# zhaoyuhsin/Edge-Guided-Near-Eye-Image-Analysis-for-Head-Mounted-Displays

Hardware: AMD Instinct MI355X
Metric: eye-frames/sec (320x240): inference edge+seg (value), +fit, exact fp32, and train fwd+bwd at 1 MI355X (higher is better)
Workload: dtype f32 tensors; inference products split into f16 hi/lo pairs (3 f16 MFMAs per product, 22-bit significand), f32 accumulate (`exact_fp32`: every product on the f32 MFMA); `train`: bf16 storage, f32 accumulate, f32 master weights (and an f32-storage leg)

## Files before the change

edge-guided-near-eye-image-analysis-for-head-mounted-displays_amd/_lib.py:

```python
import ctypes as C
import os

_HERE = os.path.dirname(os.path.abspath(__file__))
LIB_PATH = os.environ.get("EGNE_LIB") or os.path.join(_HERE, "csrc", "libegne_hip.so")

MAXSEG, MAXGROUP = 8, 3
ACT_NONE, ACT_RELU, ACT_LEAKY = 0, 1, 2

c_fp = C.c_void_p


class Seg(C.Structure):
    _fields_ = [("ptr", c_fp), ("pix_stride", C.c_int64), ("ch_off", C.c_int32), ("Cp", C.c_int32),
                ("scale", c_fp), ("shift", c_fp), ("act_in", C.c_int32), ("presplit", C.c_int32)]


class ConvDesc(C.Structure):
    _fields_ = [("B", C.c_int32), ("H", C.c_int32), ("W", C.c_int32), ("Ho", C.c_int32), ("Wo", C.c_int32),
                ("kh", C.c_int32), ("kw", C.c_int32), ("stride", C.c_int32),
                ("pad_h", C.c_int32), ("pad_w", C.c_int32), ("pad_mode", C.c_int32),
                ("ngroups", C.c_int32), ("dil", C.c_int32 * MAXGROUP),
                ("nseg", C.c_int32), ("seg", Seg * MAXSEG),
                ("Ktot", C.c_int32), ("CoutP", C.c_int32),
                ("w", c_fp), ("bias", c_fp), ("act", C.c_int32),
                ("post_scale", c_fp), ("post_shift", c_fp),
                ("residual", c_fp), ("res_pix_stride", C.c_int64), ("res_ch_off", C.c_int32),
                ("out", c_fp), ("out_pix_stride", C.c_int64), ("out_ch_off", C.c_int32),
                ("Cout_store", C.c_int32),
                ("stats_ws", c_fp), ("stats_nchunk", C.c_int32),
                ("pool_out", c_fp), ("pool_pix_stride", C.c_int64), ("pool_ch_off", C.c_int32),
                ("dyn_scale", C.c_void_p), ("absmax_out", C.c_void_p), ("dtype", C.c_int32),
                ("out_split", C.c_int32), ("out_split_scale", C.c_float), ("ovf_flag", C.c_void_p), ("f16_products", C.c_int32),
                ("mask_y", C.c_void_p), ("mask_pix_stride", C.c_int64), ("mask_ch_off", C.c_int32), ("mask_act", C.c_int32), ("mask_sums", C.c_void_p)]


class Dst(C.Structure):
    _fields_ = [("out", C.c_void_p), ("out_pix_stride", C.c_int64), ("out_ch_off", C.c_int32), ("C", C.c_int32), ("CoutP", C.c_int32),
                ("wfrag", C.c_void_p), ("residual", C.c_void_p), ("res_pix_stride", C.c_int64), ("res_ch_off", C.c_int32),
                ("mask_y", C.c_void_p), ("mask_pix_stride", C.c_int64), ("mask_ch_off", C.c_int32), ("act", C.c_int32),
                ("sums", C.c_void_p), ("res_pixels", C.c_int64)]


MAXDST = 6


class ConvQuery(C.Structure):
    _fields_ = [("dtype", C.c_int32), ("B", C.c_int32), ("H", C.c_int32), ("W", C.c_int32),
                ("kh", C.c_int32), ("kw", C.c_int32), ("stride", C.c_int32), ("pad_h", C.c_int32), ("pad_w", C.c_int32), ("pad_mode", C.c_int32),
                ("ngroups", C.c_int32), ("dil", C.c_int32 * MAXGROUP), ("nseg", C.c_int32),
                ("seg_C", C.c_int32 * MAXSEG), ("seg_Cp", C.c_int32 * MAXSEG), ("seg_ch_off", C.c_int32 * MAXSEG), ("seg_pix_stride", C.c_int64 * MAXSEG),
                ("seg_affine", C.c_int32 * MAXSEG), ("seg_planar", C.c_int32), ("seg_presplit", C.c_int32),
                ("Cout", C.c_int32), ("Cout_store", C.c_int32), ("dst_Cp", C.c_int32), ("dst_ch_off", C.c_int32), ("dst_pix_stride", C.c_int64),
                ("act", C.c_int32), ("has_post", C.c_int32), ("has_residual", C.c_int32), ("res_pix_stride", C.c_int64), ("res_ch_off", C.c_int32),
                ("split", C.c_int32), ("split1", C.c_int32), ("split_c4", C.c_int32), ("train", C.c_int32), ("dyn_scales", C.c_int32),
                ("is_dgrad", C.c_int32), ("want_stats", C.c_int32), ("want_pool", C.c_int32), ("pool_Cp", C.c_int32), ("pool_pix_stride", C.c_int64),
                ("want_scores", C.c_int32), ("up_add", C.c_int32), ("narrow_bf16_ok", C.c_int32), ("f16_products", C.c_int32), ("f16_storage", C.c_int32)]


class ConvChoice(C.Structure):
    _fields_ = [("kind", C.c_int32), ("name", C.c_char * 32), ("tail_frames", C.c_int32), ("fused_stats", C.c_int32), ("fused_pool", C.c_int32),
                ("small_ws_floats", C.c_int64)]


class BdcnTailDesc(C.Structure):
    _fields_ = [("B", C.c_int32), ("H", C.c_int32), ("W", C.c_int32),
                ("s", c_fp * 5), ("s1", c_fp * 5), ("h", C.c_int32 * 5), ("w", C.c_int32 * 5),
                ("stride", C.c_int32 * 5), ("crop", C.c_int32 * 5), ("up", c_fp * 5),
                ("fuse_w", c_fp), ("fuse_b", c_fp), ("out", c_fp * 11), ("edge_thres", C.c_int32)]


class LossDesc(C.Structure):
    _fields_ = [("B", C.c_int32), ("H", C.c_int32), ("W", C.c_int32),
                ("logits", c_fp), ("pix_stride", C.c_int64), ("ch_off", C.c_int32),
                ("target", c_fp), ("spatWts", c_fp), ("distMap", c_fp), ("cond", c_fp),
                ("pupil_center", c_fp), ("elNorm", c_fp), ("elOut", c_fp), ("alpha", C.c_float),
                ("grid_x", c_fp), ("grid_y", c_fp),
                ("partials", c_fp), ("out_terms", c_fp), ("pred_c", c_fp), ("elPred", c_fp),
                ("mask", c_fp), ("op_nchw", c_fp), ("coef", c_fp), ("dtype", C.c_int32),
                ("g_op_nchw", c_fp), ("g_pred_c", c_fp), ("g_elOut_up", c_fp)]


i32, i64, f32, vp = C.c_int32, C.c_int64, C.c_float, C.c_void_p
SIGNATURES = {
    "egne_conv2d_fwd": (i32, [C.POINTER(ConvDesc), vp]),
    "egne_pack_conv_weight": (i32, [vp, i32, i32, i32, i32, vp, i32, i32, vp, vp]),
    "egne_pack_conv_weight_frag": (i32, [vp, i32, i32, i32, i32, vp, i32, i32, vp, vp]),
    "egne_conv3x3_halo_supported": (i32, [C.POINTER(ConvDesc)]),
    "egne_conv3x3_halo_fwd": (i32, [C.POINTER(ConvDesc), vp]),
    "egne_conv3x3_smallcin_fwd": (i32, [C.POINTER(ConvDesc), vp, vp]),
    "egne_pack_conv_weight_f16x2": (i32, [vp, i32, i32, i32, i32, i32, i32, f32, vp, vp, vp]),
    "egne_conv2d_f16x3_fwd": (i32, [C.POINTER(ConvDesc), vp, vp, f32, f32, vp]),
    "egne_conv2d_f16x3_small_workspace_floats": (i64, [C.POINTER(ConvDesc)]),
    "egne_conv2d_f16x3_small_fwd": (i32, [C.POINTER(ConvDesc), vp, vp, f32, f32, vp, i64, vp]),
    "egne_pack_conv_weight_f16frag": (i32, [vp, i32, i32, i32, i32, i32, i32, f32, vp, vp, vp]),
    "egne_conv3x3_halo_f16_fwd": (i32, [C.POINTER(ConvDesc), vp, vp, f32, f32, vp]),
    "egne_conv1x1_3x3_fused_f16_fwd": (i32, [C.POINTER(ConvDesc), C.POINTER(ConvDesc), vp, vp, f32, f32, vp, vp, f32, f32, vp]),
    "egne_conv3x3c4_3x3_fused_f16_fwd": (i32, [C.POINTER(ConvDesc), C.POINTER(ConvDesc), vp, vp, f32, f32, vp, vp, f32, f32, vp]),
    "egne_msblock_dil_scores_f16_fwd": (i32, [C.POINTER(ConvDesc), vp, vp, f32, f32, vp, vp, vp, vp, i32, vp]),
    "egne_msblock_dil_f16_fwd": (i32, [C.POINTER(ConvDesc), vp, vp, f32, f32, vp]),
    "egne_conv3x3_rs_f16_fwd": (i32, [C.POINTER(ConvDesc), vp, vp, f32, f32, vp]),
    "egne_conv3x3_rw_f16_fwd": (i32, [C.POINTER(ConvDesc), vp, vp, f32, f32, vp]),
    "egne_conv1x1_pool2_f16x3_fwd": (i32, [C.POINTER(ConvDesc), vp, vp, f32, f32, vp]),
    "egne_conv1x1_f16x3_fwd": (i32, [C.POINTER(ConvDesc), vp, vp, f32, f32, vp]),
    "egne_dist_maps_workspace_bytes": (i64, [i32, i32, i32, i32]),
    "egne_dist_maps": (i32, [vp, i32, i32, i32, i32, vp, vp, vp]),
    "egne_zscore": (i32, [vp, vp, i32, i32, vp]),
    "egne_spatial_weights": (i32, [vp, i32, i32, i32, vp, vp]),
    "egne_eval_prep_workspace_bytes": (i64, [i32, i32, i32, i32, i32]),
    "egne_eval_prep": (i32, [vp, i32, i32, i32, i32, i32, i32, i32, vp, vp, vp, vp, i32, i32, vp, vp, vp, vp]),
    "egne_eval_render": (i32, [vp, i32, i32, i32, i32, i32, vp, vp, vp, i32, i32, C.c_double, i32, vp, vp, vp, vp, vp]),
    "egne_deepvog_loss_workspace_floats": (i64, [i32, i32, i32]),
    "egne_deepvog_loss_fwd": (i32, [vp, i64, i32, vp, vp, vp, i32, i32, i32, vp, vp, vp, vp, vp, vp]),
    "egne_deepvog_loss_bwd": (i32, [vp, i64, i32, vp, vp, vp, i32, i32, i32, vp, vp, vp, vp, i64, i32, vp]),
    "egne_affine_act": (i32, [vp, i64, i32, vp, i64, i32, i32, i64, vp, vp, i32, vp]),
    "egne_augment": (i32, [vp, vp, vp, vp, vp, vp, vp, vp, i32, i32, i32, vp]),
    "egne_conv3x3_smallcin_f16_fwd": (i32, [C.POINTER(ConvDesc), vp, vp, f32, f32, vp]),
    "egne_pack_conv3x3_c4_weight_f16": (i32, [vp, i32, i32, i32, f32, vp, vp, vp]),
    "egne_conv1x1_ms_f16x3_fwd": (i32, [C.POINTER(ConvDesc), vp, vp, f32, f32, vp]),
    "egne_pack_conv1x1_weight_f16x2_map": (i32, [vp, i32, i32, vp, i32, i32, f32, vp, vp, vp]),
    "egne_conv2d_f16x3_big_fwd": (i32, [C.POINTER(ConvDesc), vp, f32, f32, vp]),
    "egne_pack_conv_weight_f16img": (i32, [vp, i32, i32, i32, i32, i32, i32, f32, vp, vp]),
    "egne_conv2d_f16_big1_fwd": (i32, [C.POINTER(ConvDesc), vp, f32, f32, vp]),
    "egne_conv2d_f16_big1_supported": (i32, [C.POINTER(ConvDesc)]),
    "egne_pack_conv_weight_f16img1": (i32, [vp, i32, i32, i32, i32, i32, i32, f32, vp, vp]),
    "egne_pack_conv1x1_weight_f16": (i32, [vp, i32, i32, vp, i32, i32, f32, vp, vp, vp]),
    "egne_absmax": (i32, [vp, i64, i32, i32, i64, vp, vp]),
    "egne_absmax_f16": (i32, [vp, i64, i32, i32, i64, vp, vp]),
    "egne_norm_stats_workspace_bytes": (i64, [i32, i32, i32, i32]),
    "egne_norm_stats": (i32, [vp, i64, i32, i32, i32, i32, i32, f32, vp, vp, vp, vp, vp, vp]),
    "egne_norm_stats_finish": (i32, [vp, i32, i32, i32, i32, f32, vp, vp, vp]),
    "egne_norm_stats_finish_moments": (i32, [vp, i32, i32, i32, i32, f32, vp, vp, vp, vp, vp]),
    "egne_affine_inplace": (i32, [vp, i64, i32, i32, i64, vp, vp, vp]),
    "egne_affine": (i32, [vp, i64, i32, vp, i64, i32, i32, i64, vp, vp, vp]),
    "egne_avgpool2": (i32, [vp, i64, i32, vp, i64, i32, i32, i32, i32, i32, vp]),
    "egne_norm_act_pool2": (i32, [vp, i64, i32, vp, vp, i32, vp, i64, i32, i32, i32, i32, i32, vp]),
    "egne_maxpool2": (i32, [vp, i64, i32, vp, i64, i32, i32, i32, i32, i32, i32, i32, i32, vp]),
    "egne_maxpool2_f16": (i32, [vp, i64, i32, vp, i64, i32, i32, i32, i32, i32, i32, i32, i32, vp]),
    "egne_maxpool2_split": (i32, [vp, i64, i32, vp, i64, i32, i32, i32, i32, i32, i32, i32, i32, vp]),
    "egne_upsample2x": (i32, [vp, i64, i32, vp, i64, i32, i32, i32, i32, i32, vp]),
    "egne_upsample2x_nearest": (i32, [vp, i64, i32, vp, i64, i32, i32, i32, i32, i32, vp]),
    "egne_upsample2x_nearest_bwd": (i32, [vp, i64, i32, vp, i64, i32, i32, i32, i32, i32, vp]),
    "egne_nchw_to_nhwc": (i32, [vp, i32, i32, i32, i32, vp, i64, i32, i32, vp]),
    "egne_nhwc_to_nchw": (i32, [vp, i64, i32, i32, i32, i32, i32, vp, vp]),
    "egne_bdcn_stage_scores": (i32, [C.POINTER(vp), i32, i64, i64, vp, vp, vp, vp, vp, vp, vp, vp, vp]),
    "egne_bdcn_tail": (i32, [C.POINTER(BdcnTailDesc), vp]),
    "egne_loss_workspace_floats": (i64, [i32, i32, i32]),
    "egne_loss_fwd": (i32, [C.POINTER(LossDesc), vp]),
    "egne_ellipse_head_act": (i32, [vp, i32, i32, vp]),
    "egne_selu_inplace": (i32, [vp, i64, vp]),
    "egne_spatial_mean": (i32, [vp, i64, i32, i32, i32, i32, vp, vp]),
    "egne_softmax3": (i32, [vp, i64, i32, vp, i64, i32, i32, i64, vp]),
    "egne_adain": (i32, [vp, i64, i32, i32, vp, vp, i64, i32, vp, i64, i32, i32, i32, f32, vp]),
    "egne_conf_loss": (i32, [vp, i32, vp, i32, i32, i32, f32, vp, vp]),
    "egne_loss_bwd": (i32, [C.POINTER(LossDesc), vp, vp, i64, i32, vp, vp]),
    "egne_act_bwd_bias_workspace_bytes": (i64, [i64, i32]),
    "egne_act_bwd_bias": (i32, [vp, i64, i32, vp, i64, i32, i32, i32, i64, vp, i32, i32, vp, vp]),
    "egne_act_bwd_bias_absmax": (i32, [vp, i64, i32, vp, i64, i32, i32, i32, i64, vp, i32, i32, vp, vp, vp]),
    "egne_act_norm_bwd": (i32, [vp, i64, i32, vp, i64, i32, i32, vp, vp, vp, i64, i32, vp, i64, i32, i32, i32, i32, i32, i32, vp, vp, vp, i32, vp, i32, vp]),
    "egne_bn_act_bwd": (i32, [vp, i64, i32, i32, vp, vp, vp, vp, i64, i32, i32, i32, i32, i32, vp, i64, i32, vp, vp, vp, vp, i32, vp, i32, vp, vp]),
    "egne_zero_many": (i32, [vp, i32, i64, vp]),
    "egne_pair_bias_bwd_workspace_bytes": (i64, [i32, i32]),
    "egne_pair_bias_bwd": (i32, [vp, i64, i32, i32, i32, i32, i32, vp, vp, i32, i32, vp, vp, vp, vp]),
    "egne_norm_bwd_workspace_bytes": (i64, [i32, i32, i32, i32]),
    "egne_norm_pool2_bwd": (i32, [vp, i64, i32, vp, vp, vp, i64, i32, i32, i32, i32, i32, i32, vp, i64, i32, i32, vp, vp, vp]),
    "egne_norm_bwd_store": (i32, [vp, i64, i32, vp, vp, vp, vp, i64, i32, i32, i32, i32, i32, i32, vp, i64, i32, vp, vp, vp,
                                  i32, vp, vp]),
    "egne_norm_bwd": (i32, [vp, i64, i32, vp, vp, vp, vp, i64, i32, i32, i32, i32, i32, i32, vp, i64, i32, vp, vp, vp,
                            i32, vp, vp]),
    "egne_avgpool2_bwd": (i32, [vp, i64, i32, vp, i64, i32, i32, i32, i32, i32, vp]),
    "egne_upsample2x_bwd": (i32, [vp, i64, i32, vp, i64, i32, i32, i32, i32, i32, vp]),
    "egne_upsample2x_bwd_store": (i32, [vp, i64, i32, vp, i64, i32, i32, i32, i32, i32, vp]),
    "egne_ellipse_head_act_bwd": (i32, [vp, vp, i32, i32, vp]),
    "egne_selu_bwd": (i32, [vp, vp, i64, vp]),
    "egne_softmax3_bwd": (i32, [vp, i64, i32, vp, i64, i32, vp, i64, i32, i64, vp]),
    "egne_adain_bwd": (i32, [vp, i64, i32, i32, vp, i64, i32, vp, i64, i32, vp, i64, i32, vp, vp, i64, i32, i32, i32, f32, vp]),
    "egne_reflect_pad_bwd": (i32, [vp, i64, i32, i32, i32, vp, i64, i32, i32, i32, i32, i32, vp]),
    "egne_spatial_mean_bwd": (i32, [vp, i32, vp, i64, i32, i32, i32, i32, vp]),
    "egne_conf_loss_bwd": (i32, [vp, i32, vp, i32, i32, i32, vp, vp, i32, vp]),
    "egne_conv2d_wgrad_splits": (i32, [C.POINTER(ConvDesc)]),
    "egne_conv2d_wgrad_workspace_bytes": (i64, [C.POINTER(ConvDesc)]),
    "egne_conv2d_wgrad": (i32, [C.POINTER(ConvDesc), vp, i64, i32, i32, i32, vp, C.POINTER(vp), vp, vp]),
# ... 66 lines not shown
```

edge-guided-near-eye-image-analysis-for-head-mounted-displays_amd/csrc/common.h:

```cpp
#pragma once
#include <hip/hip_runtime.h>
#include <cstdarg>
#include <cstdio>
#include <mutex>
#include <unordered_map>
#include "../../include/egne_hip.h"

static __device__ __attribute__((aligned(256), used)) float egne_zero_page[64] = {0};

typedef __bf16 egne_bf16;
typedef float egne_f32x4 __attribute__((ext_vector_type(4)));
typedef __bf16 egne_bf16x4 __attribute__((ext_vector_type(4)));
typedef __bf16 egne_bf16x8 __attribute__((ext_vector_type(8)));

__device__ __forceinline__ egne_f32x4 ld4(const float* p) { return *(const egne_f32x4*)p; }
__device__ __forceinline__ egne_f32x4 ld4(const egne_bf16* p) { return __builtin_convertvector(*(const egne_bf16x4*)p, egne_f32x4); }
__device__ __forceinline__ void st4(float* p, egne_f32x4 v) { *(egne_f32x4*)p = v; }
__device__ __forceinline__ void st4(egne_bf16* p, egne_f32x4 v) { *(egne_bf16x4*)p = __builtin_convertvector(v, egne_bf16x4); }
__device__ __forceinline__ float ld1(const float* p) { return *p; }
__device__ __forceinline__ float ld1(const egne_bf16* p) { return (float)*p; }
__device__ __forceinline__ void st1(float* p, float v) { *p = v; }
__device__ __forceinline__ void st1(egne_bf16* p, float v) { *p = (egne_bf16)v; }
template <typename T> struct egne_vt { static constexpr int N = 4; };
template <> struct egne_vt<egne_bf16> { static constexpr int N = 8; };
template <int N> struct egne_fv { float v[N]; };
__device__ __forceinline__ egne_fv<4> ldv(const float* p) {
  const egne_f32x4 t = *(const egne_f32x4*)p;
  return egne_fv<4>{{t[0], t[1], t[2], t[3]}};
}
__device__ __forceinline__ egne_fv<8> ldv(const egne_bf16* p) {
  typedef unsigned u4_ __attribute__((ext_vector_type(4)));
  const u4_ w = *(const u4_*)p;
  egne_fv<8> r;
#pragma unroll
  for (int i = 0; i < 4; ++i) {
    r.v[2 * i] = __builtin_bit_cast(float, w[i] << 16);
    r.v[2 * i + 1] = __builtin_bit_cast(float, w[i] & 0xffff0000u);
  }
  return r;
}
__device__ __forceinline__ void stv(float* p, const egne_fv<4>& a) { *(egne_f32x4*)p = egne_f32x4{a.v[0], a.v[1], a.v[2], a.v[3]}; }
__device__ __forceinline__ void stv(egne_bf16* p, const egne_fv<8>& a) {
  const egne_f32x4 lo = {a.v[0], a.v[1], a.v[2], a.v[3]}, hi = {a.v[4], a.v[5], a.v[6], a.v[7]};
  const egne_bf16x4 l = __builtin_convertvector(lo, egne_bf16x4), h = __builtin_convertvector(hi, egne_bf16x4);
  *(egne_bf16x8*)p = egne_bf16x8{l[0], l[1], l[2], l[3], h[0], h[1], h[2], h[3]};
}
typedef unsigned egne_u32x4 __attribute__((ext_vector_type(4)));
template <typename T> __device__ __forceinline__ egne_u32x4 ldraw(const T* p) { return *(const egne_u32x4*)p; }
__device__ __forceinline__ egne_fv<4> unpackv(const float*, egne_u32x4 w) {
  return egne_fv<4>{{__builtin_bit_cast(float, w[0]), __builtin_bit_cast(float, w[1]), __builtin_bit_cast(float, w[2]), __builtin_bit_cast(float, w[3])}};
}
__device__ __forceinline__ egne_fv<8> unpackv(const egne_bf16*, egne_u32x4 w) {
  egne_fv<8> r;
#pragma unroll
  for (int i = 0; i < 4; ++i) {
    r.v[2 * i] = __builtin_bit_cast(float, w[i] << 16);
    r.v[2 * i + 1] = __builtin_bit_cast(float, w[i] & 0xffff0000u);
  }
  return r;
}
template <int N> __device__ __forceinline__ egne_fv<N> ldf(const float* p) {
  egne_fv<N> r;
#pragma unroll
  for (int i = 0; i < N; i += 4) { const egne_f32x4 t = *(const egne_f32x4*)(p + i); r.v[i] = t[0]; r.v[i + 1] = t[1]; r.v[i + 2] = t[2]; r.v[i + 3] = t[3]; }
  return r;
}
template <int N> __device__ __forceinline__ egne_fv<N> fv_fill(float x) {
  egne_fv<N> r;
#pragma unroll
  for (int i = 0; i < N; ++i) r.v[i] = x;
  return r;
}
template <typename T> __device__ __forceinline__ const T* zero_page() { return (const T*)egne_zero_page; }

#ifdef EGNE_NO_OVF_CHECK
__device__ __forceinline__ bool egne_nonfinite(float) { return false; }
__device__ __forceinline__ bool egne_nonfinite64(double) { return false; }
#else
__device__ __forceinline__ bool egne_nonfinite(float v) { return __builtin_amdgcn_classf(v, 0x207); }
__device__ __forceinline__ bool egne_nonfinite64(double v) { return !__builtin_isfinite(v); }
#endif
__device__ __forceinline__ bool egne_ovf_row(int y, int H) { return y % 3 == 1 || y == H - 1; }
__device__ __forceinline__ void egne_ovf_commit(bool bad, unsigned* flag) {
  if (flag && bad) atomicOr(flag, 1u);
}

namespace egne {

char* err_buf();

inline int fail(int code, const char* fmt, ...) {
  va_list ap;
  va_start(ap, fmt);
  vsnprintf(err_buf(), 512, fmt, ap);
  va_end(ap);
  return code;
}

inline bool fp32_storage(const egne_conv_desc& d) {
  for (int i = 0; i < d.nseg && i < EGNE_MAXSEG; ++i)
    if (d.seg[i].presplit != 0) return false;
  return d.out_split == 0;
}

inline int check_launch(const char* what) {
  hipError_t e = hipGetLastError();
  if (e != hipSuccess) return fail(EGNE_ERR_LAUNCH, "%s: %s", what, hipGetErrorString(e));
  return EGNE_OK;
}

inline bool raise_lds(const void* kern, size_t bytes) {
  static std::mutex mu;
  static std::unordered_map<const void*, size_t> have;
  std::lock_guard<std::mutex> g(mu);
  auto it = have.find(kern);
  if (it != have.end() && it->second >= bytes) return true;
  if (hipFuncSetAttribute(kern, hipFuncAttributeMaxDynamicSharedMemorySize, (int)bytes) != hipSuccess) {
    (void)hipGetLastError();
    return false;
  }
  have[kern] = bytes;
  return true;
}

#define EGNE_REQUIRE(cond, ...) \
  do { if (!(cond)) return ::egne::fail(EGNE_ERR_ARG, __VA_ARGS__); } while (0)

bool halo3_supported(const egne_conv_desc& d);
int halo3_launch(const egne_conv_desc& d, hipStream_t st);

bool wgrad_halo_supported(const egne_conv_desc& d, long long gzs);
int wgrad_halo_splits(const egne_conv_desc& d);
int wgrad_halo_launch(const egne_conv_desc& d, const float* gz, long long gzs, int gzo, float* ws, hipStream_t st);
int wgrad_halo_f16_launch(const egne_conv_desc& d, const float* gz, long long gzs, int gzo, const unsigned* gz_dyn, float* ws, hipStream_t st);

bool wgrad3x3_bf16_supported(const egne_conv_desc& d, long long gzs);
int wgrad3x3_bf16_splits(const egne_conv_desc& d);
int wgrad3x3_bf16_launch(const egne_conv_desc& d, const egne_bf16* gz, long long gzs, int gzo, float* ws, hipStream_t st);
bool wgrad1x1_bf16_supported(const egne_conv_desc& d, long long gzs);
int wgrad1x1_bf16_splits(const egne_conv_desc& d);
int wgrad1x1_bf16_launch(const egne_conv_desc& d, const egne_bf16* gz, long long gzs, int gzo, float* ws, hipStream_t st);

int msdil_ps_launch(const egne_conv_desc& d, const void* fhi, const void* flo, float a_scale, float w_scale, const float* score_w,
                    const float* score_c, float* s0, float* s1, int accumulate, hipStream_t st);

bool msdil1_wanted(const egne_conv_desc& d);
int msdil1_launch(const egne_conv_desc& d, const void* fhi, float a_scale, float w_scale, const float* score_w, const float* score_c,
                  float* s0, float* s1, int accumulate, hipStream_t st);

inline int cdiv(long long a, long long b) { return (int)((a + b - 1) / b); }

}
```

edge-guided-near-eye-image-analysis-for-head-mounted-displays_amd/csrc/msblock_dil_ps_f16.hip:

```cpp
#include "common.h"
#include <type_traits>

typedef float f32x4 __attribute__((ext_vector_type(4)));
typedef _Float16 h8 __attribute__((ext_vector_type(8)));
typedef unsigned u32x4 __attribute__((ext_vector_type(4)));
typedef __attribute__((address_space(3))) void* lds_ptr;

namespace {
__device__ int g_pdbg = 0;
__device__ unsigned long long g_pstamps[256 * 8 * 4];

constexpr int TW = 32, TH = 8;
constexpr int D0 = 4, D1 = 8, D2 = 12, DMAX = 12;
constexpr int SWMAX = TW + 2 * DMAX, NPXMAX = TH * SWMAX;
constexpr int PLANE = NPXMAX * 32 + 32;
constexpr int BUFH = 2 * PLANE;
constexpr int WBUFH = 12 * 512;
constexpr int NS = 9;
constexpr unsigned OOB = 0x80000000u;

__device__ __forceinline__ __amdgpu_buffer_rsrc_t make_rsrc(const void* base, unsigned bytes) {
  return __builtin_amdgcn_make_buffer_rsrc(const_cast<void*>(base), 0, (int)bytes, 0x00020000);
}

// ... 204 lines not shown
        for (int e = 0; e < 4; ++e) {
          const float o = ((float)resh[ph][nh * 4 + e] + (float)resl[ph][nh * 4 + e]) * inv_a;
          v[e] = fmaxf(acc[0][ph][nh][e] * out_scale + bq[0][nh][e], 0.f) + fmaxf(acc[1][ph][nh][e] * out_scale + bq[1][nh][e], 0.f) +
                 fmaxf(acc[2][ph][nh][e] * out_scale + bq[2][nh][e], 0.f) + o;
          sc[0][ph] += v[e] * cwq[0][nh][e];
          sc[1][ph] += v[e] * cwq[1][nh][e];
          if (nh == 0 && e == 0) ovf_bad |= egne_nonfinite(acc[0][ph][nh][e] + acc[1][ph][nh][e] + acc[2][ph][nh][e] + o);
        }
        if (p.out) {
          const int n = nh * 16 + 4 * kg;
          const int oo = (okp && n < p.Cout_store) ? (pix * (int)p.out_pix_stride + p.out_ch_off + n) * 4 : (int)OOB;
          __builtin_amdgcn_raw_buffer_store_b128(__builtin_bit_cast(u32x4, v), rout, oo, 0, 0);
        }
      }
    }
    if (score_w) {
#pragma unroll
      for (int h = 0; h < 2; ++h)
#pragma unroll
        for (int ph = 0; ph < 2; ++ph) {
          float t = sc[h][ph];
          t += __shfl_xor(t, 16);
          t += __shfl_xor(t, 32);
          sc[h][ph] = t;
        }
      const int h = kg >> 1, ph = kg & 1;
      const float v = h ? (ph ? sc[1][1] : sc[1][0]) : (ph ? sc[0][1] : sc[0][0]);
      if (sdst) *sdst = v + (accumulate ? sprev : lconst[160 + h]);
    }
  };

  __syncthreads();
  using I0 = std::integral_constant<int, 0>;
  using I1 = std::integral_constant<int, 1>;
  using I2 = std::integral_constant<int, 2>;
  if (nmine > 0) {
    const Tile t0 = decode(tile_at(0));
    dma_weights(I0{});
    dma_weights(I1{});
    issue_strip(t0, true, I0{});
    issue_strip(t0, true, I1{});
    issue_strip(t0, true, I2{});
    write_strip(0, I0{});
    issue_strip(t0, true, std::integral_constant<int, 3>{});
    asm volatile("s_waitcnt vmcnt(%0)" :: "n"(NI1 + NI2 + NI0) : "memory");
  }
  lds_barrier();
  for (int i = 0; i < nmine; ++i) {
    const Tile tl = decode(tile_at(i));
    const bool nx_on = i + 1 < nmine;
    const Tile nx = decode(tile_at(nx_on ? i + 1 : i));
    [&]<int... Ss>(std::integer_sequence<int, Ss...>) {
      (([&] {
        constexpr int S = Ss, S2 = (S + 2) % NS, S3 = (S + 3) % NS, S4 = (S + 4) % NS;
        const int q = 9 * i + S;
        dma_weights(std::integral_constant<int, S2>{});
        if constexpr (S == NS - 1) score_prefetch(tl);
        if constexpr (S + 1 < NS) write_strip(q + 1, std::integral_constant<int, S + 1>{});
        else if (nx_on) write_strip(q + 1, I0{});
        if constexpr (S + 4 < NS) issue_strip(tl, true, std::integral_constant<int, S4>{});
        else issue_strip(nx, nx_on, std::integral_constant<int, S4>{});
        compute_strip(q, std::integral_constant<int, S>{});
        if constexpr (S == NS - 1) epilogue(tl);
        stamp(t_work);
        asm volatile("s_waitcnt vmcnt(%0)" :: "n"(ni_of(S3 % 3) + 2 + ni_of(S4 % 3)) : "memory");
        lds_barrier();
        stamp(t_wait);
      }()), ...);
    }(std::make_integer_sequence<int, NS>{});
  }
  egne_ovf_commit(ovf_bad, p.ovf_flag);
  if ((dbg & 64) && lane == 0) {
    unsigned long long* o = g_pstamps + ((long long)blockIdx.x * 8 + wave) * 4;
    o[0] = t_work; o[1] = t_wait; o[2] = nmine; o[3] = 0;
  }
}

}

namespace egne {
int msdil_ps_launch(const egne_conv_desc& d, const void* fhi, const void* flo, float a_scale, float w_scale, const float* score_w,
                    const float* score_c, float* s0, float* s1, int accumulate, hipStream_t st) {
  if (msdil1_wanted(d)) return msdil1_launch(d, fhi, a_scale, w_scale, score_w, score_c, s0, s1, accumulate, st);
  const int tiles_x = (d.W + TW - 1) / TW, tiles_y = (d.H + TH - 1) / TH;
  const int ntiles = tiles_x * tiles_y * d.B;
  constexpr size_t lds = ((size_t)2 * BUFH + 2 * WBUFH) * sizeof(_Float16) + 162 * sizeof(float) + 18 * 64 * sizeof(int) + WBUFH * sizeof(_Float16);
  static_assert(lds <= 163840, "LDS budget");
  const float os = 1.0f / (a_scale * w_scale), inv_a = 1.0f / a_scale;
  const bool split = tiles_x > 2 && d.W >= TW * (tiles_x - 1) + 12;
  auto go = [&](auto npc) -> int {
    constexpr int NP = decltype(npc)::value;
    static bool once = hipFuncSetAttribute((const void*)msdil_ps_kernel<false, NP>, hipFuncAttributeMaxDynamicSharedMemorySize, (int)lds) == hipSuccess &&
                       hipFuncSetAttribute((const void*)msdil_ps_kernel<true, NP>, hipFuncAttributeMaxDynamicSharedMemorySize, (int)lds) == hipSuccess;
    if (!once) return egne::fail(EGNE_ERR_LAUNCH, "msblock_dil (split-pair input): cannot raise the dynamic LDS limit to %zu", lds);
    if (split) {
      const int nt_in = (tiles_x - 2) * tiles_y * d.B, nt_b = 2 * tiles_y * d.B;
      hipLaunchKernelGGL((msdil_ps_kernel<true, NP>), dim3(nt_in < 256 ? nt_in : 256), dim3(512), lds, st, d, (const _Float16*)fhi, (const _Float16*)flo,
                         inv_a, os, tiles_x, tiles_y, nt_in, 1, score_w, score_c, s0, s1, accumulate);
      static const bool only_interior = getenv("EGNE_MSDIL_ONLY_INTERIOR") != nullptr;
      if (!only_interior) hipLaunchKernelGGL((msdil_ps_kernel<false, NP>), dim3(nt_b < 256 ? nt_b : 256), dim3(512), lds, st, d, (const _Float16*)fhi,
                                             (const _Float16*)flo, inv_a, os, tiles_x, tiles_y, nt_b, 2, score_w, score_c, s0, s1, accumulate);
    } else {
      hipLaunchKernelGGL((msdil_ps_kernel<false, NP>), dim3(ntiles < 256 ? ntiles : 256), dim3(512), lds, st, d, (const _Float16*)fhi, (const _Float16*)flo,
                         inv_a, os, tiles_x, tiles_y, ntiles, 0, score_w, score_c, s0, s1, accumulate);
    }
    return EGNE_OK;
  };
  const int rc = d.f16_products == 1 ? go(std::integral_constant<int, 1>{}) : go(std::integral_constant<int, 3>{});
  if (rc != EGNE_OK) return rc;
  return egne::check_launch("egne_msblock_dil_f16_fwd (split-pair input)");
}
}

extern "C" int egne_msdil_ps_debug(int dbg, void* out_stamps) {
  if (hipMemcpyToSymbol(HIP_SYMBOL(g_pdbg), &dbg, sizeof(int)) != hipSuccess) return -2;
  if (out_stamps && hipMemcpyFromSymbol(out_stamps, HIP_SYMBOL(g_pstamps), sizeof(unsigned long long) * 256 * 8 * 4) != hipSuccess) return -2;
  return 0;
}
```

include/egne_hip.h:

```cpp
#ifndef EGNE_HIP_H
#define EGNE_HIP_H

#include <stdint.h>

#ifdef __cplusplus
extern "C" {
#endif

#define EGNE_MAXSEG 8
#define EGNE_MAXGROUP 3

typedef enum {
  EGNE_OK = 0,
  EGNE_ERR_ARG = -1,
  EGNE_ERR_LAUNCH = -2,
  EGNE_ERR_NODEVICE = -3
} egne_status;

typedef enum { EGNE_ACT_NONE = 0, EGNE_ACT_RELU = 1, EGNE_ACT_LEAKY = 2 } egne_act;

typedef struct {
  const float* ptr;
  int64_t pix_stride;
  int32_t ch_off;
  int32_t Cp;
  const float* scale;
  const float* shift;
  int32_t act_in;
  int32_t presplit;
} egne_seg;

typedef struct {
  int32_t B, H, W;
  int32_t Ho, Wo;
  int32_t kh, kw, stride;
  int32_t pad_h, pad_w;
  int32_t pad_mode;
  int32_t ngroups;
  int32_t dil[EGNE_MAXGROUP];
  int32_t nseg;
  egne_seg seg[EGNE_MAXSEG];
  int32_t Ktot;
  int32_t CoutP;
  const float* w;
  const float* bias;
  int32_t act;
  const float* post_scale;
  const float* post_shift;
  const float* residual;
  int64_t res_pix_stride;
  int32_t res_ch_off;
  float* out;
  int64_t out_pix_stride;
  int32_t out_ch_off;
  int32_t Cout_store;
  double* stats_ws;
  int32_t stats_nchunk;
  float* pool_out;
  int64_t pool_pix_stride;
  int32_t pool_ch_off;
  const uint32_t* dyn_scale;
  uint32_t* absmax_out;
  int32_t dtype;
  int32_t out_split;
  float out_split_scale;
  uint32_t* ovf_flag;
  int32_t f16_products;
  const void* mask_y; int64_t mask_pix_stride; int32_t mask_ch_off; int32_t mask_act;
  float* mask_sums;
} egne_conv_desc;

int egne_conv2d_fwd(const egne_conv_desc* d, void* stream);
int egne_conv3x3_bf16_sum_rows(void);

int egne_conv3x3_halo_supported(const egne_conv_desc* d);
int egne_conv3x3_halo_fwd(const egne_conv_desc* d, void* stream);
int egne_pack_conv_weight_frag(const float* w_oihw, int Cout, int Cin, int kh, int kw,
                               const int32_t* kinv, int CoutP, int Ktot, float* w_packed, void* stream);

int egne_pack_conv_weight_f16x2(const float* w_oihw, int Cout, int Cin, int kh, int kw, int CoutP, int Ktot,
                                float wscale, void* whi, void* wlo, void* stream);
int egne_conv2d_f16x3_fwd(const egne_conv_desc* d, const void* whi, const void* wlo, float a_scale,
                          float w_scale, void* stream);
int64_t egne_conv2d_f16x3_small_workspace_floats(const egne_conv_desc* d);
int egne_conv2d_f16x3_small_fwd(const egne_conv_desc* d, const void* whi, const void* wlo, float a_scale, float w_scale,
                                float* ws, int64_t ws_floats, void* stream);

int egne_pack_conv_weight_f16img(const float* w_oihw, int Cout, int Cin, int kh, int kw, int BN, int Ktot, float wscale,
                                 void* wimg, void* stream);
int egne_conv2d_f16x3_big_fwd(const egne_conv_desc* d, const void* wimg, float a_scale, float w_scale, void* stream);
int egne_pack_conv_weight_f16img1(const float* w_oihw, int Cout, int Cin, int kh, int kw, int BN, int Ktot, float wscale,
                                  void* wimg, void* stream);
int egne_conv2d_f16_big1_supported(const egne_conv_desc* d);
int egne_conv2d_f16_big1_fwd(const egne_conv_desc* d, const void* wimg, float a_scale, float w_scale, void* stream);

int egne_pack_conv_weight_f16frag(const float* w_oihw, int Cout, int Cin, int kh, int kw, int CoutP, int Ktot,
                                  float wscale, void* fhi, void* flo, void* stream);
int egne_conv3x3_halo_f16_fwd(const egne_conv_desc* d, const void* fhi, const void* flo, float a_scale,
                              float w_scale, void* stream);

int egne_msblock_dil_f16_fwd(const egne_conv_desc* d, const void* fhi, const void* flo, float a_scale, float w_scale,
                             void* stream);
int egne_msblock_dil_scores_f16_fwd(const egne_conv_desc* d, const void* fhi, const void* flo, float a_scale, float w_scale,
                                    const float* score_w, const float* score_c, float* s0, float* s1, int accumulate,
                                    void* stream);

int egne_conv1x1_pool2_f16x3_fwd(const egne_conv_desc* d, const void* fhi, const void* flo, float a_scale, float w_scale,
                                 void* stream);

int egne_conv3x3_rs_f16_fwd(const egne_conv_desc* d, const void* fhi, const void* flo, float a_scale, float w_scale,
                            void* stream);

int egne_conv3x3_rw_f16_fwd(const egne_conv_desc* d, const void* fhi, const void* flo, float a_scale, float w_scale,
                            void* stream);

int egne_pack_conv1x1_weight_f16(const float* w_oihw, int Cout, int Cin, const int32_t* kmap, int G, int CoutP,
                                 float wscale, void* fhi, void* flo, void* stream);
int egne_conv1x1_f16x3_fwd(const egne_conv_desc* d, const void* fhi, const void* flo, float a_scale,
                           float w_scale, void* stream);

int egne_conv1x1_3x3_fused_f16_fwd(const egne_conv_desc* d1, const egne_conv_desc* d2, const void* w1hi, const void* w1lo,
                                   float a1, float w1_scale, const void* f2hi, const void* f2lo, float a2, float w2_scale,
                                   void* stream);

int egne_conv3x3c4_3x3_fused_f16_fwd(const egne_conv_desc* d1, const egne_conv_desc* d2, const void* c4hi, const void* c4lo,
                                     float a1, float w1_scale, const void* f2hi, const void* f2lo, float a2, float w2_scale,
                                     void* stream);

int egne_pack_conv1x1_weight_f16x2_map(const float* w_oihw, int Cout, int Cin, const int32_t* kmap, int CoutP, int Ktot,
                                       float wscale, void* whi, void* wlo, void* stream);
int egne_conv1x1_ms_f16x3_fwd(const egne_conv_desc* d, const void* whi, const void* wlo, float a_scale,
                              float w_scale, void* stream);

int egne_conv3x3_smallcin_fwd(const egne_conv_desc* d, const float* w40, void* stream);

int egne_pack_conv3x3_c4_weight_f16(const float* w_oihw, int Cout, int Cin, int CoutP, float wscale, void* fhi, void* flo,
                                    void* stream);
int egne_conv3x3_smallcin_f16_fwd(const egne_conv_desc* d, const void* fhi, const void* flo, float a_scale,
                                  float w_scale, void* stream);

int egne_pack_conv_weight(const float* w_oihw, int Cout, int Cin, int kh, int kw,
                          const int32_t* kinv, int CoutP, int Ktot, float* w_packed, void* stream);

int egne_absmax(const float* x, int64_t pix_stride, int ch_off, int Cp, int64_t npix, void* out_bits, void* stream);
int egne_absmax_f16(const void* x, int64_t pix_stride, int ch_off, int Cp, int64_t npix, void* out_bits, void* stream);

int64_t egne_norm_stats_workspace_bytes(int B, int HW, int Cp, int per_sample);
int egne_norm_stats(const float* x, int64_t pix_stride, int ch_off, int Cp, int B, int HW,
                    int per_sample, float eps, float* scale, float* shift,
                    float* mean_out, float* var_out, void* ws, void* stream);

int egne_norm_stats_finish(const void* ws, int Cp, int B, int nchunk, int HW, float eps, float* scale, float* shift,
                           void* stream);
int egne_norm_stats_finish_moments(const void* ws, int Cp, int B, int nchunk, int HW, float eps, float* scale, float* shift,
                                   float* mean_out, float* var_out, void* stream);

int egne_affine_inplace(float* x, int64_t pix_stride, int ch_off, int Cp, int64_t npix,
                        const float* scale, const float* shift, void* stream);

int egne_affine(const float* x, int64_t xs, int xo, float* y, int64_t ys, int yo, int Cp, int64_t npix,
                const float* scale, const float* shift, void* stream);

int egne_avgpool2(const float* x, int64_t xs, int xo, float* y, int64_t ys, int yo,
                  int B, int H, int W, int Cp, void* stream);

int egne_norm_act_pool2(const float* x, int64_t xs, int xo, const float* scale, const float* shift, int act,
                        float* y, int64_t ys, int yo, int B, int H, int W, int Cp, void* stream);

int egne_maxpool2(const float* x, int64_t xs, int xo, float* y, int64_t ys, int yo,
                  int B, int H, int W, int Ho, int Wo, int stride, int Cp, void* stream);
int egne_maxpool2_f16(const void* x, int64_t xs, int xo, void* y, int64_t ys, int yo, int B, int H, int W, int Ho, int Wo, int stride,
                      int Cp, void* stream);

int egne_maxpool2_split(const void* x, int64_t xs, int xo, void* y, int64_t ys, int yo, int B, int H, int W, int Ho, int Wo, int stride,
                        int Cp, void* stream);

int egne_upsample2x(const float* x, int64_t xs, int xo, float* y, int64_t ys, int yo,
                    int B, int H, int W, int Cp, void* stream);

int egne_nchw_to_nhwc(const float* x, int B, int C, int H, int W, float* y, int64_t ys, int yo,
                      int Cp, void* stream);
int egne_nhwc_to_nchw(const float* x, int64_t xs, int xo, int B, int C, int H, int W, float* y,
                      void* stream);

int egne_bdcn_stage_scores(const float* const* ms, int nblk, int64_t ms_pix_stride, int64_t npix,
                           const float* wd, const float* bd, const float* ws, const float* bs,
                           const float* ws1, const float* bs1, float* s, float* s1, void* stream);

// ... 314 lines not shown
```

Before: 2100.

## Add polyphase persistent kernel for three-product dilated msblock convolution

Adds a new persistent kernel for the multi-scale dilated 3x3 block in the hi/lo f16 three-product path. It splits the input into 4x4 polyphase sub-images, so every dilation becomes a dense neighbour access. Input rows stream through an LDS ring buffer with async buffer-to-LDS loads that overlap compute, and the kernel walks work items across rows. Weights stay in LDS or registers, and the ReLU-sum, residual and score reductions are fused into the epilogue. The code adds a launch counter and makes the LDS-attribute cache per device; the price is a complex, register-heavy kernel that needs over 150 KB of LDS per block.

```diff
diff --git a/edge-guided-near-eye-image-analysis-for-head-mounted-displays_amd/_lib.py b/edge-guided-near-eye-image-analysis-for-head-mounted-displays_amd/_lib.py
--- a/edge-guided-near-eye-image-analysis-for-head-mounted-displays_amd/_lib.py
+++ b/edge-guided-near-eye-image-analysis-for-head-mounted-displays_amd/_lib.py
@@ -97,6 +97,7 @@
     "egne_conv1x1_3x3_fused_f16_fwd": (i32, [C.POINTER(ConvDesc), C.POINTER(ConvDesc), vp, vp, f32, f32, vp, vp, f32, f32, vp]),
     "egne_conv3x3c4_3x3_fused_f16_fwd": (i32, [C.POINTER(ConvDesc), C.POINTER(ConvDesc), vp, vp, f32, f32, vp, vp, f32, f32, vp]),
     "egne_msblock_dil_scores_f16_fwd": (i32, [C.POINTER(ConvDesc), vp, vp, f32, f32, vp, vp, vp, vp, i32, vp]),
+    "egne_msdil3_launches": (C.c_longlong, []),
     "egne_msblock_dil_f16_fwd": (i32, [C.POINTER(ConvDesc), vp, vp, f32, f32, vp]),
     "egne_conv3x3_rs_f16_fwd": (i32, [C.POINTER(ConvDesc), vp, vp, f32, f32, vp]),
     "egne_conv3x3_rw_f16_fwd": (i32, [C.POINTER(ConvDesc), vp, vp, f32, f32, vp]),
diff --git a/edge-guided-near-eye-image-analysis-for-head-mounted-displays_amd/csrc/common.h b/edge-guided-near-eye-image-analysis-for-head-mounted-displays_amd/csrc/common.h
--- a/edge-guided-near-eye-image-analysis-for-head-mounted-displays_amd/csrc/common.h
+++ b/edge-guided-near-eye-image-analysis-for-head-mounted-displays_amd/csrc/common.h
@@ -2,6 +2,7 @@
 #include <hip/hip_runtime.h>
 #include <cstdarg>
 #include <cstdio>
+#include <map>
 #include <mutex>
 #include <unordered_map>
 #include "../../include/egne_hip.h"
@@ -111,15 +112,21 @@
 
 inline bool raise_lds(const void* kern, size_t bytes) {
   static std::mutex mu;
-  static std::unordered_map<const void*, size_t> have;
+  static std::map<std::pair<int, const void*>, size_t> have;
   std::lock_guard<std::mutex> g(mu);
-  auto it = have.find(kern);
+  int dev = 0;
+  if (hipGetDevice(&dev) != hipSuccess) {
+    (void)hipGetLastError();
+    return false;
+  }
+  const std::pair<int, const void*> key(dev, kern);
+  auto it = have.find(key);
   if (it != have.end() && it->second >= bytes) return true;
   if (hipFuncSetAttribute(kern, hipFuncAttributeMaxDynamicSharedMemorySize, (int)bytes) != hipSuccess) {
     (void)hipGetLastError();
     return false;
   }
-  have[kern] = bytes;
+  have[key] = bytes;
   return true;
 }
 
@@ -147,6 +154,9 @@
 bool msdil1_wanted(const egne_conv_desc& d);
 int msdil1_launch(const egne_conv_desc& d, const void* fhi, float a_scale, float w_scale, const float* score_w, const float* score_c,
                   float* s0, float* s1, int accumulate, hipStream_t st);
+bool msdil3_wanted(const egne_conv_desc& d);
+int msdil3_launch(const egne_conv_desc& d, const void* fhi, const void* flo, float a_scale, float w_scale, const float* score_w,
+                  const float* score_c, float* s0, float* s1, int accumulate, hipStream_t st);
 
 inline int cdiv(long long a, long long b) { return (int)((a + b - 1) / b); }
 
diff --git a/edge-guided-near-eye-image-analysis-for-head-mounted-displays_amd/csrc/msblock_dil3_f16.hip b/edge-guided-near-eye-image-analysis-for-head-mounted-displays_amd/csrc/msblock_dil3_f16.hip
--- /dev/null
+++ b/edge-guided-near-eye-image-analysis-for-head-mounted-displays_amd/csrc/msblock_dil3_f16.hip
@@ -0,0 +1,309 @@
+#include "common.h"
+#include <atomic>
+#include <cstdlib>
+#include <type_traits>
+#include <utility>
+
+typedef float f32x4 __attribute__((ext_vector_type(4)));
+typedef _Float16 h8 __attribute__((ext_vector_type(8)));
+typedef unsigned u32x4 __attribute__((ext_vector_type(4)));
+typedef __attribute__((address_space(3))) void* lds_ptr;
+
+namespace {
+
+constexpr int TW = 16, TH = 8, HALO = 3;
+constexpr int RPX = 24, RROWS = 2 * TH + 2 * HALO;
+constexpr int ROWB = RPX * 128, RINGB = RROWS * ROWB;
+constexpr int RPIECES = ROWB / 1024;
+constexpr int WHI = 2 * 9 * 2048, WLO = 3 * 9 * 2048;
+constexpr int OFF_WH = RINGB, OFF_WL = OFF_WH + WHI, OFF_CONST = OFF_WL + WLO;
+constexpr int LDS_BYTES = OFF_CONST + 164 * 4;
+constexpr unsigned OOB = 0x80000000u;
+static_assert(LDS_BYTES <= 163840, "LDS budget");
+
+__device__ __forceinline__ __amdgpu_buffer_rsrc_t make_rsrc(const void* base, unsigned bytes) {
+  return __builtin_amdgcn_make_buffer_rsrc(const_cast<void*>(base), 0, (int)bytes, 0x00020000);
+}
+
+__device__ __forceinline__ void lds_barrier() {
+  asm volatile("s_waitcnt lgkmcnt(0)" ::: "memory");
+  __builtin_amdgcn_s_barrier();
+  asm volatile("" ::: "memory");
+}
+
+struct Tap { int g, ky, kx; };
+constexpr Tap tap_at(int i) { return Tap{i % 3, (i / 3) / 3, (i / 3) % 3}; }
+
+__global__ __launch_bounds__(512)
+void msdil3_kernel(const egne_conv_desc p, const _Float16* __restrict__ fhi, const _Float16* __restrict__ flo, float inv_a, float out_scale,
+                   int ncols, int nseg, int seg_rows, int nitems, const float* __restrict__ score_w, const float* __restrict__ score_c,
+                   float* __restrict__ s0, float* __restrict__ s1, int accumulate) {
+  extern __shared__ __attribute__((aligned(1024))) char lds[];
+  float* const lconst = (float*)(lds + OFF_CONST);
+  const int tid = threadIdx.x, lane = tid & 63;
+  const int wave = __builtin_amdgcn_readfirstlane(tid >> 6);
+  const int l15 = lane & 15, kg = lane >> 4;
+  const int H = p.H, W = p.W, Hs = H >> 2, Ws = W >> 2;
+  const egne_seg sg = p.seg[0];
+  const int pixb = (int)sg.pix_stride * 4;
+
+  if (tid < 160) {
+    const int r = tid >> 5, c = tid & 31;
+    lconst[tid] = r < 3 ? (p.bias ? p.bias[r * p.CoutP + c] : 0.f) : (score_w ? score_w[(r - 3) * 32 + c] : 0.f);
+  } else if (tid < 162) {
+    lconst[tid] = score_c ? score_c[tid - 160] : 0.f;
+  }
+  {
+    const __amdgpu_buffer_rsrc_t rwh = make_rsrc(fhi, 3u * 9u * 2u * 1024u), rwl = make_rsrc(flo, 3u * 9u * 2u * 1024u);
+    for (int k = wave; k < 90; k += 8) {
+      if (k < 36) __builtin_amdgcn_raw_ptr_buffer_load_lds(rwh, (lds_ptr)(lds + OFF_WH + k * 1024), 16, lane * 16, k * 1024, 0, 0);
+      else __builtin_amdgcn_raw_ptr_buffer_load_lds(rwl, (lds_ptr)(lds + OFF_WL + (k - 36) * 1024), 16, lane * 16, (k - 36) * 1024, 0, 0);
+    }
+  }
+  const int wl = (kg >> 1) * 1024 + ((kg & 1) * 32 + l15) * 16;
+  h8 w2[9][2];
+#pragma unroll
+  for (int t = 0; t < 9; ++t)
+#pragma unroll
+    for (int nh = 0; nh < 2; ++nh) w2[t][nh] = *(const h8*)((const char*)fhi + (18 + t) * 2048 + wl + nh * 256);
+
+  int relq[RPIECES], colq[RPIECES];
+#pragma unroll
+  for (int j = 0; j < RPIECES; ++j) {
+    const int q = 8 * j + (lane >> 3), pos = lane & 7;
+    const int t = ((pos & 3) - (q >> 1)) & 3;
+    colq[j] = q < TW + 2 * HALO ? q - HALO : -100000;
+    relq[j] = 4 * (q - HALO) * pixb + sg.ch_off * 4 + (t & 1) * 64 + ((pos >> 2) | (t & 2)) * 16;
+  }
+  int ahi[7], alo[7];
+#pragma unroll
+  for (int c0 = 0; c0 < 7; ++c0) {
+    const int q = c0 + l15, e = (q >> 1) + 2 * (kg >> 1);
+    ahi[c0] = q * 128 + ((((kg & 1) << 2) | (e & 3)) << 4);
+    alo[c0] = q * 128 + ((((kg & 1) << 2) | ((e + 1) & 3)) << 4);
+  }
+
+  const unsigned frame_in = (unsigned)H * W * (unsigned)sg.pix_stride * 4u;
+  const unsigned frame_out = (unsigned)H * W * (unsigned)p.out_pix_stride * 4u;
+  const int per = (int)gridDim.x >> 3;
+  auto item_at = [&](int i) { return ((int)gridDim.x & 7) ? (int)blockIdx.x + i * (int)gridDim.x : ((i * 8 + ((int)blockIdx.x & 7)) * per + ((int)blockIdx.x >> 3)); };
+  bool ovf_bad = false;
+
+  struct Item { int b, py, px, x0, ys, ye, nst; };
+  auto decode = [&](int it) {
+    Item r;
+    const int sgi = it % nseg; it /= nseg;
+    const int phase = it & 15; it >>= 4;
+    const int cx = it % ncols;
+    r.b = it / ncols; r.py = phase >> 2; r.px = phase & 3; r.x0 = cx * TW; r.ys = sgi * seg_rows;
+    r.ye = r.ys + seg_rows < Hs ? r.ys + seg_rows : Hs;
+    r.nst = (r.ye - r.ys + TH - 1) / TH;
+    return r;
+  };
+  auto col_offsets = [&](const Item& m, int (&offc)[RPIECES]) {
+#pragma unroll
+    for (int j = 0; j < RPIECES; ++j)
+      offc[j] = (unsigned)(m.x0 + colq[j]) < (unsigned)Ws ? relq[j] + (4 * m.x0 + m.px) * pixb : (int)OOB;
+  };
+  auto issue_rows = [&](const Item& m, const int (&offc)[RPIECES], int yf, int ringrow, int nrows) {
+    const __amdgpu_buffer_rsrc_t rin = make_rsrc(sg.ptr + (long long)m.b * H * W * sg.pix_stride, frame_in);
+    for (int k = wave; k < RPIECES * nrows; k += 8) {
+      const int r = k / RPIECES, j = k - r * RPIECES;
+      const int y = yf + r;
+      int rr = ringrow + r;
+      rr = rr >= RROWS ? rr - RROWS : rr;
+      const int oc = j == 0 ? offc[0] : (j == 1 ? offc[1] : offc[2]);
+      const int off = ((unsigned)y < (unsigned)Hs && oc != (int)OOB) ? oc + (4 * y + m.py) * W * pixb : (int)OOB;
+      __builtin_amdgcn_raw_ptr_buffer_load_lds(rin, (lds_ptr)(lds + rr * ROWB + j * 1024), 16, off, 0, 0, 0);
+    }
+  };
+  auto wrap = [](int r) { return r >= RROWS ? r - RROWS : r; };
+
+  int it = item_at(0);
+  Item cur = decode(it);
+  int offc[RPIECES];
+  col_offsets(cur, offc);
+  issue_rows(cur, offc, cur.ys - HALO, 0, TH + 2 * HALO);
+  asm volatile("s_waitcnt vmcnt(0)" ::: "memory");
+  int r0 = 0;
+
+  for (int ii = 0;; ++ii) {
+    const int itn = item_at(ii + 1);
+    const bool has_next = itn < nitems;
+    const Item nxt = decode(has_next ? itn : it);
+    int offn[RPIECES];
+    col_offsets(nxt, offn);
+    const int b = cur.b, py = cur.py, px = cur.px, x0 = cur.x0, ys = cur.ys, nst = cur.nst;
+    for (int t = 0; t < nst; ++t) {
+      const int y0 = ys + TH * t;
+      const bool last = t + 1 == nst;
+      const int rn = wrap(r0 + TH + 2 * HALO);
+      lds_barrier();
+      if (!last) issue_rows(cur, offc, y0 + TH + HALO, rn, TH);
+      else if (has_next) issue_rows(nxt, offn, nxt.ys - HALO, rn, TH);
+      const bool rowon = y0 + wave < cur.ye;
+      float* sdst = nullptr;
+      float sprev = 0.f;
+      {
+        const int y = y0 + wave, x = x0 + l15;
+        if (score_w && !(kg & 1) && y < Hs && x < Ws) sdst = ((kg >> 1) ? s1 : s0) + ((long long)b * H + 4 * y + py) * W + 4 * x + px;
+        if (sdst && accumulate) sprev = *(const volatile float*)sdst;
+      }
+      int rb[7];
+#pragma unroll
+      for (int j = 0; j < 7; ++j) {
+        const int rr = r0 + wave + j;
+        rb[j] = (rr >= RROWS ? rr - RROWS : rr) * ROWB;
+      }
+
+      f32x4 acc[3][2];
+#pragma unroll
+      for (int a = 0; a < 6; ++a) (&acc[0][0])[a] = (f32x4)(0.f);
+      h8 ah[2], al[2], wh[2][2], wo[2][2], resh, resl;
+
+      auto fetch = [&](auto ic) {
+        constexpr int I = decltype(ic)::value;
+        constexpr Tap tp = tap_at(I);
+        constexpr int d = tp.g + 1, j = 3 + (tp.ky - 1) * d, c0 = HALO + (tp.kx - 1) * d, tw = tp.g * 9 + tp.ky * 3 + tp.kx;
+        ah[I & 1] = *(const h8*)(lds + rb[j] + ahi[c0]);
+        al[I & 1] = *(const h8*)(lds + rb[j] + alo[c0]);
+#pragma unroll
+        for (int nh = 0; nh < 2; ++nh) {
+          if constexpr (tp.g < 2) wh[I & 1][nh] = *(const h8*)(lds + OFF_WH + wl + (tw * 2048 + nh * 256));
+          wo[I & 1][nh] = *(const h8*)(lds + OFF_WL + wl + (tw * 2048 + nh * 256));
+        }
+      };
+      auto multiply = [&](auto ic) {
+        constexpr int I = decltype(ic)::value;
+        constexpr Tap tp = tap_at(I);
+        if constexpr (tp.g == 0 && tp.ky == 1 && tp.kx == 1) { resh = ah[I & 1]; resl = al[I & 1]; }
+        h8 wa[2];
+#pragma unroll
+        for (int nh = 0; nh < 2; ++nh) {
+          if constexpr (tp.g < 2) wa[nh] = wh[I & 1][nh];
+          else wa[nh] = w2[tp.ky * 3 + tp.kx][nh];
+        }
+#pragma unroll
+        for (int nh = 0; nh < 2; ++nh) acc[tp.g][nh] = __builtin_amdgcn_mfma_f32_16x16x32_f16(wa[nh], al[I & 1], acc[tp.g][nh], 0, 0, 0);
+#pragma unroll
+        for (int nh = 0; nh < 2; ++nh) acc[tp.g][nh] = __builtin_amdgcn_mfma_f32_16x16x32_f16(wo[I & 1][nh], ah[I & 1], acc[tp.g][nh], 0, 0, 0);
+#pragma unroll
+        for (int nh = 0; nh < 2; ++nh) acc[tp.g][nh] = __builtin_amdgcn_mfma_f32_16x16x32_f16(wa[nh], ah[I & 1], acc[tp.g][nh], 0, 0, 0);
+      };
+
+      if (rowon) {
+      fetch(std::integral_constant<int, 0>{});
+      [&]<int... Is>(std::integer_sequence<int, Is...>) {
+        (([&] {
+          constexpr int I = Is;
+          if constexpr (I + 1 < 27) fetch(std::integral_constant<int, I + 1>{});
+          __builtin_amdgcn_sched_barrier(0);
+          multiply(std::integral_constant<int, I>{});
+          __builtin_amdgcn_sched_barrier(0);
+        }()), ...);
+      }(std::make_integer_sequence<int, 27>{});
+      }
+
+      asm volatile("s_waitcnt vmcnt(0)" ::: "memory");
+      if (last && has_next) {
+        lds_barrier();
+        issue_rows(nxt, offn, nxt.ys - HALO + TH, wrap(rn + TH), 2 * HALO);
+      }
+      if (rowon) {
+        const int y = y0 + wave, x = x0 + l15;
+        const __amdgpu_buffer_rsrc_t rout = make_rsrc(p.out ? p.out + (long long)b * H * W * p.out_pix_stride : nullptr, p.out ? frame_out : 0u);
+        f32x4 bq[3][2], cwq[2][2];
+#pragma unroll
+        for (int nh = 0; nh < 2; ++nh) {
+          const int n = nh * 16 + 4 * kg;
+#pragma unroll
+          for (int g = 0; g < 3; ++g) bq[g][nh] = *(const f32x4*)&lconst[g * 32 + n];
+#pragma unroll
+          for (int h = 0; h < 2; ++h) cwq[h][nh] = *(const f32x4*)&lconst[(3 + h) * 32 + n];
+        }
+        const bool okp = y < Hs && x < Ws;
+        const int pix = (4 * y + py) * W + 4 * x + px;
+        float sc[2];
+        sc[0] = sc[1] = 0.f;
+#pragma unroll
+        for (int nh = 0; nh < 2; ++nh) {
+          f32x4 v;
+#pragma unroll
+          for (int e = 0; e < 4; ++e) {
+            const float o = ((float)resh[nh * 4 + e] + (float)resl[nh * 4 + e]) * inv_a;
+            v[e] = fmaxf(acc[0][nh][e] * out_scale + bq[0][nh][e], 0.f) + fmaxf(acc[1][nh][e] * out_scale + bq[1][nh][e], 0.f) +
+                   fmaxf(acc[2][nh][e] * out_scale + bq[2][nh][e], 0.f) + o;
+            sc[0] += v[e] * cwq[0][nh][e];
+            sc[1] += v[e] * cwq[1][nh][e];
+            if (nh == 0 && e == 0) ovf_bad |= egne_nonfinite(acc[0][nh][e] + acc[1][nh][e] + acc[2][nh][e] + o);
+          }
+          if (p.out) {
+            const int n = nh * 16 + 4 * kg;
+            const int oo = (okp && n < p.Cout_store) ? (pix * (int)p.out_pix_stride + p.out_ch_off + n) * 4 : (int)OOB;
+            __builtin_amdgcn_raw_buffer_store_b128(__builtin_bit_cast(u32x4, v), rout, oo, 0, 0);
+          }
+        }
+        if (score_w) {
+#pragma unroll
+          for (int h = 0; h < 2; ++h) {
+            float tt = sc[h];
+            tt += __shfl_xor(tt, 16);
+            tt += __shfl_xor(tt, 32);
+            sc[h] = tt;
+          }
+          const int h = kg >> 1;
+          const float v = h ? sc[1] : sc[0];
+          if (sdst) *sdst = v + (accumulate ? sprev : lconst[160 + h]);
+        }
+      }
+      if (last && has_next) asm volatile("s_waitcnt vmcnt(0)" ::: "memory");
+      r0 = last ? rn : wrap(r0 + TH);
+    }
+    if (!has_next) break;
+    it = itn;
+    cur = nxt;
+#pragma unroll
+    for (int j = 0; j < RPIECES; ++j) offc[j] = offn[j];
+  }
+  asm volatile("s_waitcnt vmcnt(0)" ::: "memory");
+  egne_ovf_commit(ovf_bad, p.ovf_flag);
+}
+
+}
+
+static std::atomic<long long> g_msdil3_launches{0};
+
+namespace egne {
+
+bool msdil3_wanted(const egne_conv_desc& d) {
+  const char* e = getenv("EGNE_MSDIL3");
+  return !(e && atoi(e) == 0) && d.f16_products != 1 && d.seg[0].presplit == 1 && d.H % 4 == 0 && d.W % 4 == 0 && d.H >= 32 && d.W >= 64;
+}
+
+int msdil3_launch(const egne_conv_desc& d, const void* fhi, const void* flo, float a_scale, float w_scale, const float* score_w,
+                  const float* score_c, float* s0, float* s1, int accumulate, hipStream_t st) {
+  const int Hs = d.H / 4, Ws = d.W / 4;
+  const int ncols = (Ws + TW - 1) / TW;
+  int best = 1;
+  double best_t = 1e30;
+  for (int ns = 1; ns <= 4; ++ns) {
+    const int rows = ((Hs + ns - 1) / ns + TH - 1) / TH * TH;
+    if (ns > 1 && rows * (ns - 1) >= Hs) continue;
+    const long long items = (long long)d.B * ncols * 16 * ns;
+    const double t = (double)((items + 255) / 256) * (rows / TH + 1.5);
+    if (t < best_t) { best_t = t; best = ns; }
+  }
+  const int seg_rows = ((Hs + best - 1) / best + TH - 1) / TH * TH;
+  const long long nitems = (long long)d.B * ncols * 16 * best;
+  if (!egne::raise_lds((const void*)msdil3_kernel, LDS_BYTES))
+    return egne::fail(EGNE_ERR_LAUNCH, "msblock_dil (three products, polyphase form): cannot raise the dynamic LDS limit to %d", LDS_BYTES);
+  const float os = 1.0f / (a_scale * w_scale), inv_a = 1.0f / a_scale;
+  hipLaunchKernelGGL(msdil3_kernel, dim3((unsigned)(nitems < 256 ? nitems : 256)), dim3(512), LDS_BYTES, st, d, (const _Float16*)fhi,
+                     (const _Float16*)flo, inv_a, os, ncols, best, seg_rows, (int)nitems, score_w, score_c, s0, s1, accumulate);
+  g_msdil3_launches.fetch_add(1, std::memory_order_relaxed);
+  return egne::check_launch("egne_msblock_dil_f16_fwd (three products, polyphase form)");
+}
+
+}
+
+extern "C" long long egne_msdil3_launches(void) { return g_msdil3_launches.load(std::memory_order_relaxed); }
diff --git a/edge-guided-near-eye-image-analysis-for-head-mounted-displays_amd/csrc/msblock_dil_ps_f16.hip b/edge-guided-near-eye-image-analysis-for-head-mounted-displays_amd/csrc/msblock_dil_ps_f16.hip
--- a/edge-guided-near-eye-image-analysis-for-head-mounted-displays_amd/csrc/msblock_dil_ps_f16.hip
+++ b/edge-guided-near-eye-image-analysis-for-head-mounted-displays_amd/csrc/msblock_dil_ps_f16.hip
@@ -310,6 +310,7 @@
 int msdil_ps_launch(const egne_conv_desc& d, const void* fhi, const void* flo, float a_scale, float w_scale, const float* score_w,
                     const float* score_c, float* s0, float* s1, int accumulate, hipStream_t st) {
   if (msdil1_wanted(d)) return msdil1_launch(d, fhi, a_scale, w_scale, score_w, score_c, s0, s1, accumulate, st);
+  if (msdil3_wanted(d)) return msdil3_launch(d, fhi, flo, a_scale, w_scale, score_w, score_c, s0, s1, accumulate, st);
   const int tiles_x = (d.W + TW - 1) / TW, tiles_y = (d.H + TH - 1) / TH;
   const int ntiles = tiles_x * tiles_y * d.B;
   constexpr size_t lds = ((size_t)2 * BUFH + 2 * WBUFH) * sizeof(_Float16) + 162 * sizeof(float) + 18 * 64 * sizeof(int) + WBUFH * sizeof(_Float16);
diff --git a/include/egne_hip.h b/include/egne_hip.h
--- a/include/egne_hip.h
+++ b/include/egne_hip.h
@@ -104,6 +104,7 @@
 int egne_msblock_dil_scores_f16_fwd(const egne_conv_desc* d, const void* fhi, const void* flo, float a_scale, float w_scale,
                                     const float* score_w, const float* score_c, float* s0, float* s1, int accumulate,
                                     void* stream);
+long long egne_msdil3_launches(void);
 
 int egne_conv1x1_pool2_f16x3_fwd(const egne_conv_desc* d, const void* fhi, const void* flo, float a_scale, float w_scale,
                                  void* stream);
```

Result: faster. 2148 (median of 6 runs) (+2.3%).
